# HyperBitGore/deflate.hpp

Measured on AMD Instinct MI355X. Metric: GB/s deflate+inflate on 1 GiB buffer at 1/2/4/8 MI355X; ratio vs reference, higher is better.
Workload: dtype u8; 1 GPU; deflate level 2 + inflate round trip of a per-GPU 1 GiB 'repeat' corpus (SURVEY App. B), device-resident; corpus=repeat, bytes_per_gpu=1073741824, level=2, segment_bytes=32768, parallelism=shard1

## Files before the change

### deflate.hpp_amd/csrc/deflate_kernels.hip

```cpp
#include "dmx_device.h"
#include "dmx_internal.h"
#include "huff_fit.h"

namespace dmx {

constexpr int DF_NT = 1024;
constexpr int DF_CHUNK = 258;
constexpr int df_hash_bits(int seg) {
    return seg >= 32768 ? 12 : 11;
}
constexpr int DF_L3_DEPTH = 16;
constexpr uint32_t DF_L3_LONG = 16;
constexpr uint32_t DF_L3_RP = 512;
constexpr bool df_early(int seg) { return seg >= 32768; }
constexpr uint32_t EM_ALL_LITERALS = 0xFFFFFFFFu;


__device__ __forceinline__ int df_tid() {
    int t = threadIdx.x;
    asm volatile("" : "+v"(t));
    return t;
}

__device__ uint32_t block_excl_scan(uint32_t v, uint32_t* scratch, uint32_t* total) {
// ... 795 lines not shown
                            for (int j = 0; j < 4; j++)
                                x |= __builtin_amdgcn_alignbyte(data32[ip + j + 1], data32[ip + j], sp) ^
                                     __builtin_amdgcn_alignbyte(data32[iq + j + 1], data32[iq + j], sq);
                            pass = x == 0;
                        }
                        const int qb = lane_id() & ~3;
                        uint32_t pm = (uint32_t)(__ballot(pass) >> qb) & 0xFu;
                        while (pm) {
                            const int f = __builtin_ctz(pm);
                            pm &= pm - 1;
                            const uint32_t d1 = (uint32_t)__shfl((int)dk, qb + f, 64);
                            if (len_at(p, d1, ml) >= L) {
                                best = d1;
                                break;
                            }
                        }
                    }
                    if (lead) S.cand[p] = (uint16_t)best;
                }
                tok |= 1u << (p & 31);
                if (lead) S.cand[p + 1] = (uint16_t)L;
                p += L;
            }
            if (tok && lead) atomicOr(&S.tokmap[w], tok);
            if (lead) S.lasttok[t >> 2] = (uint16_t)lastp;
        };
        if (level >= 2 && (uint32_t)t < 4 * nwalk) {
            if constexpr (TERMRUN) {
                if (run_lo != RUN_NONE) parse_walk(std::true_type{});
                else parse_walk(std::false_type{});
            } else
                parse_walk(std::false_type{});
        }
        if constexpr (EARLY) asm volatile("s_waitcnt vmcnt(0)" ::: "memory");
        __syncthreads();
        DMX_PHASE(A.dbg, seg, 3);

        if (level >= 2) {
            const uint32_t sub = t & 3, c = t >> 2;
            const uint32_t hb = D + (c + 1) * CH;
            if ((uint32_t)t < 4 * (nwalk - 1) && hb < nb) {
                const uint32_t s0 = S.lasttok[c], d0 = S.cand[s0], L0 = S.cand[s0 + 1];
                const uint32_t sn = S.lasttok[c + 1];
                if (d0 != 0 && s0 + L0 == hb && L0 < 258 && sn >= hb + 2) {
                    const uint32_t Lx = matchlen4(data32, s0, s0 - d0, min(258u, sn - 1 - s0), sub);
                    const uint32_t e = s0 + Lx;
                    uint32_t q = 0;
                    if (Lx > L0) {
                        uint32_t w = e >> 5;
                        uint32_t m = S.tokmap[w] & (0xFFFFFFFFu >> (31 - (e & 31)));
                        while (!m) m = S.tokmap[--w];
                        q = w * 32 + 31 - (uint32_t)__clz(m);
                    }
                    if (Lx > L0 && sub == 0) {
                        const uint32_t dq = S.cand[q], Lq = q == e ? 0u : S.cand[q + 1];
                        const uint32_t r = q == e ? 0u : q + Lq - e;
                        const uint32_t sync = q == e ? e : q + Lq;
                        uint32_t old = 0;
                        for (uint32_t wi = s0 >> 5; wi <= (sync - 1) >> 5; wi++) {
                            const uint32_t a = max(s0, wi * 32) - wi * 32, z = min(sync, wi * 32 + 32) - wi * 32;
                            const uint32_t rm = (z >= 32 ? 0xFFFFFFFFu : ((1u << z) - 1u)) & (0xFFFFFFFFu << a);
                            old += (uint32_t)__popc(S.tokmap[wi] & rm);
                        }
                        const uint32_t nt = 1 + (r >= 3 ? 1u : r);
                        if (nt < old) {
                            uint32_t nb0 = 0, nb1 = 0;
                            if (r) {
                                atomicOr(&S.tokmap[e >> 5], 1u << (e & 31));
                                if (r == 2) atomicOr(&S.tokmap[(e + 1) >> 5], 1u << ((e + 1) & 31));
                            }
                            S.cand[s0 + 1] = (uint16_t)Lx;
                            if (r >= 3) {
                                S.cand[e] = (uint16_t)dq;
                                S.cand[e + 1] = (uint16_t)r;
                            } else if (r) {
                                S.cand[e] = 0;
                                if (r == 2) S.cand[e + 1] = 0;
                            }
                            for (uint32_t wi = s0 >> 5; wi <= (sync - 1) >> 5; wi++) {
                                const uint32_t a = max(s0, wi * 32) - wi * 32, z = min(sync, wi * 32 + 32) - wi * 32;
                                const uint32_t rm = (z >= 32 ? 0xFFFFFFFFu : ((1u << z) - 1u)) & (0xFFFFFFFFu << a);
                                nb0 = (s0 >> 5) == wi ? 1u << (s0 & 31) : 0u;
                                nb1 = (r && (e >> 5) == wi ? 1u << (e & 31) : 0u) |
                                      (r == 2 && ((e + 1) >> 5) == wi ? 1u << ((e + 1) & 31) : 0u);
                                atomicAnd(&S.tokmap[wi], ~rm | nb0 | nb1);
                            }
                        }
                    }
                }
            }
            __syncthreads();
        }

        bool by_word = false;
        if constexpr (TERMRUN) {
            static_assert(NMAP == DF_NT, "one token-start bitmap word per thread");
            by_word = run_lo != RUN_NONE;
        }
        if (by_word) {
            const uint32_t m = S.tokmap[t];
            const uint4* const c4 = reinterpret_cast<const uint4*>(S.cand + 32 * t);
            uint32_t nz = 0;
#pragma unroll
            for (int k = 0; k < 4; k++) {
                const uint4 v = c4[k];
                const uint32_t x[4] = {v.x, v.y, v.z, v.w};
#pragma unroll
                for (int j = 0; j < 4; j++) {
                    nz |= ((x[j] & 0xFFFFu) ? 1u : 0u) << (8 * k + 2 * j);
                    nz |= ((x[j] >> 16) ? 1u : 0u) << (8 * k + 2 * j + 1);
                }
            }
            const uint32_t mt = m & nz, lt = m & ~nz;
            const uint32_t chain = lt & (lt << 1) & (lt << 2) & (lt << 3);
            uint32_t ws = lt & ~(lt << 1);
#pragma unroll
            for (int i = 0; i < 10; i++) ws |= (ws << 3) & chain;
            const uint32_t val = ((uint32_t)__popc(m) << 16) | ((uint32_t)__popc(mt) + (uint32_t)__popc(ws));
            const uint32_t inc = wave_incl_scan(val);
            uint32_t* const sc = S.scan + DF_NT / 64;
            if ((t & 63) == 63) sc[t >> 6] = inc;
            __syncthreads();
            uint32_t ex = inc - val, tot = 0;
#pragma unroll
            for (int i = 0; i < DF_NT / 64; i++) {
                const uint32_t x = sc[i];
                if (i < (t >> 6)) ex += x;
                tot += x;
            }
            DMX_PHASE(A.dbg, seg, 15);
            if ((tot >> 16) == nb - D) {
                if (t == 0) A.ntok[seg] = EM_ALL_LITERALS;
            } else {
                uint32_t* dst = A.tok + seg * (uint64_t)A.tok_stride + (ex & 0xFFFFu);
                const uint32_t* const sw = reinterpret_cast<const uint32_t*>(&S);
                const uint32_t cbase = (uint32_t)(reinterpret_cast<const uint32_t*>(S.cand) - sw) + 16 * (uint32_t)t;
                const uint32_t dbase = (uint32_t)(data32 - sw) + 8 * (uint32_t)t;
                uint32_t all = mt | ws;
                while (all) {
                    uint32_t b[4], lo[4], hi[4];
                    bool on[4];
#pragma unroll
                    for (int i = 0; i < 4; i++) {
                        on[i] = all != 0;
                        b[i] = on[i] ? (uint32_t)__builtin_ctz(all) : 0u;
                        all &= all - 1;
                        const uint32_t at = (mt >> b[i]) & 1u ? cbase + (b[i] >> 1) : dbase + (b[i] >> 2);
                        lo[i] = sw[at];
                        hi[i] = sw[at + 1];
                    }
#pragma unroll
                    for (int i = 0; i < 4; i++) {
                        if (on[i]) {
                            const bool mat = (mt >> b[i]) & 1u;
                            const uint32_t v = __builtin_amdgcn_alignbyte(hi[i], lo[i], mat ? 2 * (b[i] & 1) : b[i] & 3);
                            const uint32_t x = lt >> b[i], c = 1 + ((x >> 1) & 1u) + ((x >> 1) & (x >> 2) & 1u);
                            *dst++ = mat ? 0x80000000u | (((v >> 16) - 3) << 16) | ((v & 0xFFFFu) - 1)
                                         : (v & (0xFFFFFFu >> (24 - 8 * c))) | (c << 24);
                        }
                    }
                }
                if (t == 0) A.ntok[seg] = tot & 0xFFFFu;
            }
        } else {
            TokRange tr;
            uint32_t tr_total;
            {
                const uint32_t c = t < NMAP ? (uint32_t)__popc(S.tokmap[t]) : 0u;
                uint32_t tot;
                const uint32_t ex = block_excl_scan(c, S.scan, &tot);
                if (t < NMAP) S.mmap[t] = ex;
                __syncthreads();
                tr_total = tot;
                const uint32_t K = (tot + DF_NT - 1) / DF_NT;
                const uint32_t first = min((uint32_t)t * K, tot);
                tr.n = min(first + K, tot) - first;
                uint32_t lo = 0, hi = NMAP;
                while (hi - lo > 1) {
                    const uint32_t mid = (lo + hi) >> 1;
                    if (S.mmap[mid] <= first) lo = mid;
                    else hi = mid;
                }
                tr.w = lo;
                const uint32_t m = S.tokmap[lo];
                uint32_t b = 0, k = tr.n ? first - S.mmap[lo] : 0u;
    #pragma unroll
                for (uint32_t sh = 16; sh >= 1; sh >>= 1) {
                    const uint32_t c = (uint32_t)__popc((m >> b) & ((1u << sh) - 1u));
                    const bool up = k >= c;
                    b += up ? sh : 0u;
                    k -= up ? c : 0u;
                }
                tr.m = m & (0xFFFFFFFFu << b);
            }
            DMX_PHASE(A.dbg, seg, 15);
            const bool all_lit = tr_total == nb - D;
            if (all_lit) {
                if (t == 0) A.ntok[seg] = EM_ALL_LITERALS;
            } else {
                auto walk = [&](auto emit) {
                    uint32_t w = tr.w, m = tr.m, lit = 0, nl = 0;
                    for (uint32_t i = 0; i < tr.n; i++) {
                        const uint32_t p = next_tok(S.tokmap, w, m);
                        const uint32_t d = S.cand[p];
                        if (d) {
                            if (nl) emit(lit | (nl << 24));
                            nl = 0;
                            lit = 0;
                            emit(0x80000000u | ((uint32_t)(S.cand[p + 1] - 3) << 16) | (d - 1));
                        } else {
                            lit |= (uint32_t)data_byte(data32, p) << (8 * nl);
                            if (++nl == 3) {
                                emit(lit | (3u << 24));
                                nl = 0;
                                lit = 0;
                            }
                        }
                    }
                    if (nl) emit(lit | (nl << 24));
                };
                uint32_t nw = 0;
                walk([&](uint32_t) { nw++; });
                uint32_t wtot;
                const uint32_t woff = block_excl_scan(nw, S.scan, &wtot);
                uint32_t* const dst = A.tok + seg * (uint64_t)A.tok_stride + woff;
                uint32_t j = 0;
                walk([&](uint32_t v) { dst[j++] = v; });
                if (t == 0) A.ntok[seg] = wtot;
            }
        }
        DMX_PHASE(A.dbg, seg, 11);
        if constexpr (!EARLY) {
            __syncthreads();
            staged = df_prefetch_next<SEG, BATCH, DICT, PIPE>(A, seg, data32);
        }
        DMX_PHASE(A.dbg, seg, 10);
    }
}

template <int SEG, bool L3, bool BATCH, bool DICT, bool PIPE = false>
__device__ __forceinline__ void deflate_segments(const DeflateArgs& A, DfSmem<SEG>& S) {
    constexpr bool EARLY = DfSmem<SEG>::EARLY;
    uint32_t staged = 0;
    uint32_t iw = 0;
    if constexpr (EARLY) {
        const int t = df_tid();
        if (t < 64) S.buf[t >> 5][SEG / 4 + (t & 31)] = 0;
    }
    uint64_t first = 0;
    if constexpr (PIPE) first = static_cast<const DeflatePipeArgs&>(A).seg_first;
    const auto end = [&]() -> uint64_t {
        if constexpr (PIPE) return static_cast<const DeflatePipeArgs&>(A).seg_end;
        else return df_nseg<BATCH>(A);
    };
    for (uint64_t seg = first + blockIdx.x; seg < end(); seg += gridDim.x) {
        deflate_segment<SEG, L3, BATCH, DICT, PIPE>(A, S, seg, staged, iw);
        if constexpr (EARLY) {
            df_lds_barrier();
            iw = (uint32_t)DfSmem<SEG>::BW - iw;
        } else
            __syncthreads();
    }
}
template <int SEG, bool L3, bool BATCH = false, bool DICT = false>
__global__ __launch_bounds__(DF_NT) void k_deflate_segments(DeflateArgs A) {
    static_assert(!BATCH && !DICT, "a batch runs k_deflate_segments_batch");
    __shared__ DfSmem<SEG> S;
    deflate_segments<SEG, L3, false, false>(A, S);
}
template <bool L3, bool BATCH = false>
__global__ __launch_bounds__(DF_NT) __attribute__((amdgpu_waves_per_eu(8, 8))) void k_deflate_segments16(DeflateArgs A) {
    static_assert(!BATCH, "a batch runs k_deflate_segments16_batch");
    __shared__ DfSmem<16384> S;
    deflate_segments<16384, L3, false, false>(A, S);
}
template <int SEG, bool L3, bool DICT = false>
__global__ __launch_bounds__(DF_NT) void k_deflate_segments_batch(DeflateBatchArgs A) {
    __shared__ DfSmem<SEG> S;
    deflate_segments<SEG, L3, true, DICT>(A, S);
}
template <bool L3>
__global__ __launch_bounds__(DF_NT) __attribute__((amdgpu_waves_per_eu(8, 8))) void k_deflate_segments16_batch(DeflateBatchArgs A) {
    __shared__ DfSmem<16384> S;
    deflate_segments<16384, L3, true, false>(A, S);
}
template <bool L3>
__global__ __launch_bounds__(DF_NT) __attribute__((amdgpu_num_vgpr(52))) void k_deflate_segments_pipe(DeflatePipeArgs A) {
    __shared__ DfSmem<32768> S;
    deflate_segments<32768, L3, false, false, true>(A, S);
}

constexpr int EM_NW = 4;
constexpr int EM_FLUSH = 256;
constexpr int EM_STG = 576;
constexpr int EM_LIT = 288, EM_SYM = 320;

struct EmWave {
    union {
        uint32_t freq[EM_SYM];
        uint32_t stg[EM_STG];
    };
    uint32_t code[EM_SYM];
    uint8_t len[EM_SYM];
    uint16_t rk[EM_SYM];
    uint32_t prefreq[20];
    uint32_t precode[20];
    uint8_t prelen[24];
    uint32_t hcnt[6][20];
    uint32_t lcnt[6][16];
    uint32_t kpre[2][20];
    uint32_t start[2][16];
    uint32_t next[2][16];
};
static_assert(3 * sizeof(EmWave) <= 163840 - 140320, "three emission waves fit beside a front workgroup's LDS");

struct EmCodes {
    uint32_t dyn_tok, fix_tok;
    uint32_t nlit, ndist;
};

__device__ __forceinline__ uint32_t em_slot(int c, int lane) { return c < 5 ? 64 * c + lane : EM_LIT + lane; }
__device__ __forceinline__ bool em_valid(int c, int lane) { return c < 5 ? 64 * c + lane < 286 : lane < 30; }

__device__ EmCodes em_build_codes(EmWave& W) {
    const int lane = lane_id();
    const uint64_t lt = (1ull << lane) - 1ull;
    uint32_t Fl = 0, nzl = 0, hil = 0;
    for (int c = 0; c < 5; c++) {
        const uint32_t f = em_valid(c, lane) ? W.freq[em_slot(c, lane)] : 0u;
        Fl += f;
        const uint64_t b = __ballot(f != 0);
        nzl += (uint32_t)__popcll(b);
        if (b) hil = 64 * c + 64 - (uint32_t)__clzll(b);
    }
    Fl = wave_sum(Fl);
    const uint32_t f5 = lane < 30 ? W.freq[EM_LIT + lane] : 0u;
    const uint32_t Fd = wave_sum(f5);
    const uint64_t bd = __ballot(f5 != 0);
    const uint32_t nzd = (uint32_t)__popcll(bd), hid = bd ? 64 - (uint32_t)__clzll(bd) : 0u;
    for (int c = 0; c < 6; c++) {
        const uint32_t f = em_valid(c, lane) ? W.freq[em_slot(c, lane)] : 0u;
        const uint32_t F = c < 5 ? Fl : Fd;
        const uint32_t L0 = init_len(f, F, c < 5 ? DF_LIT_MAXBITS : DF_DIST_MAXBITS);
        const uint32_t k0 = L0 ? 2 * L0 + init_half(f, F, L0) : 0u;
        uint32_t mine = 0, w0 = 0;
#pragma unroll
        for (int k = 2; k <= 2 * DF_LIT_MAXBITS + 1; k++) {
            const uint64_t b = __ballot(k0 == (uint32_t)k);
            mine = lane == k ? (uint32_t)__popcll(b) : mine;
            w0 = k0 == (uint32_t)k ? (uint32_t)__popcll(b & lt) : w0;
        }
        if (lane < 20) W.hcnt[c][lane] = mine;
        W.rk[64 * c + lane] = (uint16_t)(k0 | (w0 << 5));
    }
    wave_sync();
    {
        const int a = lane >= 32 ? 1 : 0, k = lane & 31;
        uint32_t v = 0;
        if (k < 20) {
            if (a) v = W.hcnt[5][k];
            else v = W.hcnt[0][k] + W.hcnt[1][k] + W.hcnt[2][k] + W.hcnt[3][k] + W.hcnt[4][k];
        }
        uint32_t inc = v;
#pragma unroll
        for (int d = 1; d < 32; d <<= 1) {
            const uint32_t u = __shfl_up(inc, d, 64);
            if (k >= d) inc += u;
        }
        if (k < 20) W.kpre[a][k] = inc - v;
        uint32_t cnt[17];
        cnt[0] = cnt[16] = 0;
        const uint32_t nz = a ? nzd : nzl;
#pragma unroll
        for (int L = 1; L <= 15; L++) {
            const uint32_t x = (2 * L + 1 < 20) ? (uint32_t)__shfl(v, (a << 5) + 2 * L, 64) +
                                                      (uint32_t)__shfl(v, (a << 5) + 2 * L + 1, 64)
                                                : 0u;
            cnt[L] = nz > 1 ? x : (L == 1 ? 2u : 0u);
        }
        if (nz > 1) fit_classes(cnt, a ? DF_DIST_MAXBITS : DF_LIT_MAXBITS);
        if (k == 0) {
            uint32_t st = 0, code = 0;
#pragma unroll
            for (int L = 1; L <= 15; L++) {
                W.start[a][L] = st;
                st += cnt[L];
                code = (code + cnt[L - 1]) << 1;
                W.next[a][L] = code;
            }
        }
    }
    wave_sync();
    for (int c = 0; c < 6; c++) {
        const int a = c == 5 ? 1 : 0;
        const bool sym = em_valid(c, lane);
        const uint32_t nz = a ? nzd : nzl;
        uint32_t L = 0;
        if (sym) {
            const uint32_t s = c < 5 ? 64 * c + lane : (uint32_t)lane;
            if (nz > 1) {
                if (W.freq[em_slot(c, lane)]) {
                    const uint32_t r = W.rk[64 * c + lane], k0 = r & 31;
                    uint32_t q = (r >> 5) + W.kpre[a][k0];
                    for (int c2 = 0; c2 < c && !a; c2++) q += W.hcnt[c2][k0];
#pragma unroll
                    for (int l = 1; l <= 15; l++) L += q >= W.start[a][l] ? 1u : 0u;
                }
            } else {
                const uint32_t u = a ? hid : hil;
                L = (s == (u ? u - 1 : 0u) || s == (u <= 1 ? 1u : 0u)) ? 1u : 0u;
            }
            W.len[em_slot(c, lane)] = (uint8_t)L;
        }
        uint32_t mine = 0, wl = 0;
#pragma unroll
        for (int k = 1; k <= DF_LIT_MAXBITS; k++) {
            const uint64_t b = __ballot(L == (uint32_t)k);
            wl = L == (uint32_t)k ? (uint32_t)__popcll(b & lt) : wl;
            mine = lane == k ? (uint32_t)__popcll(b) : mine;
        }
        if (lane < 16) W.lcnt[c][lane] = mine;
        W.rk[64 * c + lane] = (uint16_t)wl;
    }
    wave_sync();
    uint32_t dyn = 0, fix = 0, hl = 0, hd = 0;
    for (int c = 0; c < 6; c++) {
        const int a = c == 5 ? 1 : 0;
        const bool sym = em_valid(c, lane);
        const uint32_t L = sym ? W.len[em_slot(c, lane)] : 0u;
        if (sym) {
            const uint32_t s = c < 5 ? 64 * c + lane : (uint32_t)lane;
            uint32_t code = 0;
            if (L) {
                uint32_t cc = W.next[a][L] + W.rk[64 * c + lane];
                for (int c2 = 0; c2 < c && !a; c2++) cc += W.lcnt[c2][L];
                code = (L << 16) | bitrev(cc, L);
            }
            W.code[em_slot(c, lane)] = code;
            const uint32_t f = W.freq[em_slot(c, lane)];
            const uint32_t ex = a ? dist_extra(s) : (s > 256 ? len_extra(s) : 0u);
            dyn += f * (L + ex);
            fix += f * ((a ? 5u : fixed_lit_len(s)) + ex);
        }
        const uint64_t used = __ballot(L != 0);
        if (used) {
            const uint32_t h = 64 - (uint32_t)__clzll(used);
            if (a) hd = h;
            else hl = 64 * c + h;
        }
    }
    wave_sync();
    EmCodes r;
    r.dyn_tok = wave_sum(dyn);
    r.fix_tok = wave_sum(fix);
    r.nlit = max(257u, hl);
    r.ndist = max(1u, hd);
    return r;
}

__device__ __forceinline__ void em_put(uint32_t* stg, uint32_t pos, uint64_t pat, uint32_t n) {
    if (!n) return;
    const uint32_t wi = pos >> 5, sh = pos & 31;
    const uint64_t lo = pat << sh;
    atomicOr(&stg[wi], (uint32_t)lo);
    if (sh + n > 32) atomicOr(&stg[wi + 1], (uint32_t)(lo >> 32));
    if (sh + n > 64) atomicOr(&stg[wi + 2], (uint32_t)(pat >> (64 - sh)));
}

__device__ __forceinline__ uint64_t em_pattern(const EmWave& W, uint32_t v, uint32_t cnt, uint32_t& n, bool raw) {
    uint64_t pat = 0;
    n = 0;
    if (!raw && (v >> 31)) {
        const uint32_t L = ((v >> 16) & 0xFFu) + 3, d = (v & 0x7FFFu) + 1;
        const uint32_t ls = len_sym(L), ds = dist_sym(d);
        const uint32_t lc = W.code[ls], dc = W.code[EM_LIT + ds];
        pat = lc & 0xFFFFu;
        n = lc >> 16;
        pat |= (uint64_t)(L - len_base(ls)) << n;
        n += len_extra(ls);
        pat |= (uint64_t)(dc & 0xFFFFu) << n;
        n += dc >> 16;
        pat |= (uint64_t)(d - dist_base(ds)) << n;
        n += dist_extra(ds);
        return pat;
    }
#pragma unroll
    for (uint32_t i = 0; i < 4u; i++) {
        if (i < cnt) {
            const uint32_t c = W.code[(v >> (8 * i)) & 0xFFu];
            pat |= (uint64_t)(c & 0xFFFFu) << n;
            n += c >> 16;
        }
    }
    return pat;
}

__device__ __forceinline__ void em_flush(uint32_t* stg, uint32_t* dst, uint32_t nw) {
    const int lane = lane_id();
#pragma unroll 2
    for (uint32_t i = lane; i < nw; i += 64) dst[i] = stg[i];
    wave_sync();
    const uint32_t part = stg[nw];
    wave_sync();
#pragma unroll 2
    for (uint32_t i = lane; i <= nw + 1; i += 64) stg[i] = i == 0 ? part : 0u;
    wave_sync();
}

#define EM_PHASE(dbg, seg, slot)                                                          \
    do {                                                                                  \
        if ((dbg) && lane_id() == 0) (dbg)[(seg) * kPhaseSlots + (slot)] = __builtin_amdgcn_s_memtime(); \
    } while (0)

struct EmSrc {
    const uint32_t* inw;
    const uint32_t* tok;
    uint64_t in_words_end;
    uint32_t mis;
    uint32_t nb;
    uint32_t ntok;
    bool raw;
    __device__ uint32_t raw_word(uint32_t k) const {
        const uint32_t x = 4 * k + mis;
        const uint32_t a = inw[x >> 2];
        const uint32_t b = (x >> 2) + 1 < in_words_end ? inw[(x >> 2) + 1] : 0u;
        return mis ? __builtin_amdgcn_alignbyte(b, a, x & 3) : a;
    }
    __device__ void load4(uint32_t blk, uint32_t (&v)[4]) const {
        const uint32_t i0 = blk * 256 + 4 * lane_id();
#pragma unroll
        for (int j = 0; j < 4; j++) v[j] = 0;
        if (raw) {
#pragma unroll
            for (int j = 0; j < 4; j++)
                if (i0 + j < ntok) v[j] = raw_word(i0 + j);
        } else if (i0 + 3 < ntok) {
            const uint4 q = *reinterpret_cast<const uint4*>(tok + i0);
            v[0] = q.x, v[1] = q.y, v[2] = q.z, v[3] = q.w;
        } else {
#pragma unroll
            for (int j = 0; j < 4; j++)
                if (i0 + j < ntok) v[j] = tok[i0 + j];
        }
    }
    __device__ uint32_t count_of(uint32_t v, uint32_t idx) const {
        if (raw) return min(4u, nb - 4 * idx);
        return (v >> 31) ? 0u : (v >> 24) & 3u;
    }
};
template <bool RAW>
__device__ EmSrc em_src(const DeflateArgs& A, uint64_t fseg, const uint8_t* inb, uint64_t tail, uint32_t nb) {
    EmSrc s;
    s.mis = (uint32_t)(reinterpret_cast<uintptr_t>(inb) & 3);
    s.inw = reinterpret_cast<const uint32_t*>(inb - s.mis);
    s.in_words_end = (tail + s.mis + 3) / 4;
    s.nb = nb;
    s.raw = RAW || A.ntok[fseg] == EM_ALL_LITERALS;
    s.ntok = s.raw ? (nb + 3) / 4 : A.ntok[fseg];
    s.tok = s.raw ? nullptr : A.tok + fseg * (uint64_t)A.tok_stride;
    return s;
}

__device__ __forceinline__ uint32_t em_stored_hdr(uint32_t q, bool fin, uint32_t len) {
    return q == 0 ? (fin ? 1u : 0u) : q == 1 ? len & 0xFFu : q == 2 ? (len >> 8) & 0xFFu
         : q == 3 ? ~len & 0xFFu : (~len >> 8) & 0xFFu;
}

template <int SEG, bool RAW, bool BATCH>
__device__ void em_segment(const DeflateArgs& A, EmWave& W, uint64_t seg) {
    static_assert(!BATCH || SEG <= 32768, "a batch does not pair front segments into 64 KiB blocks");
    constexpr uint32_t NH = SEG > 32768 ? 2u : 1u;
    constexpr uint32_t HB = (uint32_t)SEG / NH;
    const int lane = lane_id();
    EM_PHASE(A.dbg, seg, 4);
    const DfSegAddr sa = df_seg_addr<SEG, BATCH>(A, seg);
    const uint32_t nb = sa.nb;
    const uint32_t np = (nb + HB - 1) / HB;
    const bool is_final = sa.is_last && A.final_last;
    uint32_t* const slot = reinterpret_cast<uint32_t*>(A.slots + seg * (uint64_t)A.slot_bytes);
    auto part = [&](uint32_t h) {
        return em_src<RAW>(A, seg * NH + h, sa.src + (uint64_t)h * HB, sa.tail - (uint64_t)h * HB, min(HB, nb - h * HB));
    };
    const uint32_t nsto = nb > 65535u ? 2u : 1u;
    const uint32_t n1 = nsto == 2 ? 32768u : nb;
    const uint64_t stored_bytes = 5ull * nsto + nb + (is_final ? 0 : 5);

    if (A.level != 0) {
        for (int i = lane; i < EM_SYM; i += 64) W.freq[i] = 0;
        wave_sync();
        for (uint32_t h = 0; h < np; h++) {
            const EmSrc S = part(h);
            const uint32_t nblk = (S.ntok + 255) / 256;
            for (uint32_t blk = 0; blk < nblk; blk++) {
                uint32_t v[4];
                S.load4(blk, v);
#pragma unroll
                for (int j = 0; j < 4; j++) {
                    const uint32_t idx = blk * 256 + 4 * lane + j;
                    if (idx >= S.ntok) continue;
                    if (!S.raw && (v[j] >> 31)) {
                        atomicAdd(&W.freq[len_sym(((v[j] >> 16) & 0xFFu) + 3)], 1u);
                        atomicAdd(&W.freq[EM_LIT + dist_sym((v[j] & 0x7FFFu) + 1)], 1u);
                    } else {
                        const uint32_t cnt = S.count_of(v[j], idx);
#pragma unroll
                        for (uint32_t i = 0; i < 4u; i++)
                            if (i < cnt) atomicAdd(&W.freq[(v[j] >> (8 * i)) & 0xFFu], 1u);
                    }
                }
            }
        }
        wave_sync();
        if (lane == 0) atomicAdd(&W.freq[256], 1u);
        wave_sync();
        EM_PHASE(A.dbg, seg, 5);
        const EmCodes ec = em_build_codes(W);
        EM_PHASE(A.dbg, seg, 6);
        const uint32_t nlit = ec.nlit, ndist = ec.ndist, nall = nlit + ndist;
        auto seqv = [&](uint32_t i) -> uint32_t { return i < nlit ? W.len[i] : W.len[EM_LIT + i - nlit]; };
        uint64_t rm[5];
        if (lane < 20) W.prefreq[lane] = 0;
#pragma unroll
        for (int c = 0; c < 5; c++) {
            const uint32_t i = 64 * c + lane;
            bool start = false;
            if (i < nall) start = i == 0 || i == nlit || seqv(i - 1) != seqv(i);
            rm[c] = __ballot(start);
        }
        wave_sync();
        for (int c = 0; c < 5; c++) {
            uint32_t rl = 0;
            if ((rm[c] >> lane) & 1) {
                const uint32_t i = 64 * c + lane;
                uint32_t j = nall;
                const uint64_t m = lane < 63 ? rm[c] & (~0ull << (lane + 1)) : 0ull;
                if (m) j = 64 * c + (uint32_t)__builtin_ctzll(m);
                else
                    for (int c2 = 4; c2 > c; c2--)
                        if (rm[c2]) j = 64 * c2 + (uint32_t)__builtin_ctzll(rm[c2]);
                rl = min(j, nall) - i;
                const uint32_t v = seqv(i);
                const RunPlan p = plan_run(v, rl);
                if (p.n18) atomicAdd(&W.prefreq[18], p.n18);
                if (p.n17) atomicAdd(&W.prefreq[17], p.n17);
                if (p.n16) atomicAdd(&W.prefreq[16], p.n16);
                if (p.nlit) atomicAdd(&W.prefreq[v], p.nlit);
            }
            W.rk[64 * c + lane] = (uint16_t)rl;
        }
        wave_sync();
        wave_build_lengths64(W.prefreq, 19, DF_PRE_MAXBITS, W.prelen);
        wave_sync();
        wave_assign_codes(W.prelen, 19, W.precode);
        wave_sync();
        const uint32_t pv = lane < 19 ? W.prelen[kPerm[lane]] : 0u;
        const uint64_t nzp = __ballot(pv != 0u);
        const uint32_t hclen = max(4u, nzp ? 64u - (uint32_t)__clzll(nzp) : 0u);
        uint32_t rtot = 0;
        for (int c = 0; c < 5; c++) {
            const uint32_t rl = W.rk[64 * c + lane];
            uint32_t b = 0;
            if (rl) {
                const uint32_t v = seqv(64 * c + lane);
                const RunPlan p = plan_run(v, rl);
                b = p.n18 * (W.prelen[18] + 7) + p.n17 * (W.prelen[17] + 3) + p.n16 * (W.prelen[16] + 2) +
                    p.nlit * W.prelen[v];
            }
            const uint32_t inc = wave_incl_scan(b);
            W.rk[64 * c + lane] = (uint16_t)(rl ? rtot + inc - b : 0xFFFFu);
            rtot += __shfl(inc, 63, 64);
        }
        wave_sync();
        const uint32_t hdr_bits = 14 + 3 * hclen + rtot;
        EM_PHASE(A.dbg, seg, 7);

        const uint64_t dyn_bits = 3ull + hdr_bits + ec.dyn_tok;
        const uint64_t fix_bits = 3ull + ec.fix_tok;
        const bool use_dyn = dyn_bits <= fix_bits;
        const uint64_t bits = use_dyn ? dyn_bits : fix_bits;
        const uint64_t hbytes = is_final ? (bits + 7) / 8 : (bits + 3 + 7) / 8 + 4;
        if (hbytes < stored_bytes) {
            if (!use_dyn) {
                for (int s = lane; s < EM_SYM; s += 64)
                    W.code[s] = s < EM_LIT ? (s < 286 ? (fixed_lit_len(s) << 16) | fixed_lit_code(s) : 0u)
                                           : (s - EM_LIT < 30 ? (5u << 16) | bitrev(s - EM_LIT, 5) : 0u);
            }
#pragma unroll 3
            for (int i = lane; i < EM_STG; i += 64) W.stg[i] = 0;
            wave_sync();
            if (lane == 0) {
                uint64_t h = (is_final ? 1u : 0u) | ((use_dyn ? 2u : 1u) << 1);
                if (use_dyn) h |= ((uint64_t)(nlit - 257) << 3) | ((uint64_t)(ndist - 1) << 8) | ((uint64_t)(hclen - 4) << 13);
                em_put(W.stg, 0, h, use_dyn ? 17 : 3);
            }
            if (use_dyn) {
                if (lane < (int)hclen) em_put(W.stg, 17 + 3 * lane, pv, 3);
                const uint32_t rb = 17 + 3 * hclen;
                for (int c = 0; c < 5; c++) {
                    const uint32_t ro = W.rk[64 * c + lane];
                    if (ro == 0xFFFFu) continue;
                    const uint32_t i = 64 * c + lane;
                    const uint32_t v = seqv(i);
                    uint32_t j = nall;
                    const uint64_t m = lane < 63 ? rm[c] & (~0ull << (lane + 1)) : 0ull;
                    if (m) j = 64 * c + (uint32_t)__builtin_ctzll(m);
                    else
                        for (int c2 = 4; c2 > c; c2--)
                            if (rm[c2]) j = 64 * c2 + (uint32_t)__builtin_ctzll(rm[c2]);
                    const RunPlan p = plan_run(v, min(j, nall) - i);
                    uint32_t pos = rb + ro;
                    auto put = [&](uint32_t sym, uint32_t extra, uint32_t xb) {
                        const uint32_t pc = W.precode[sym];
                        const uint32_t l = pc >> 16;
                        em_put(W.stg, pos, (uint64_t)(pc & 0xFFFFu) | ((uint64_t)extra << l), l + xb);
                        pos += l + xb;
                    };
                    if (v == 0) {
                        for (uint32_t q = 0; q < p.n18; q++) put(18, (q + 1 == p.n18 ? p.last18 : 138) - 11, 7);
                        if (p.n17) put(17, p.r17 - 3, 3);
                        for (uint32_t q = 0; q < p.nlit; q++) put(0, 0, 0);
                    } else {
                        put(v, 0, 0);
                        for (uint32_t q = 0; q < p.n16; q++) put(16, (q + 1 == p.n16 ? p.last16 : 6) - 3, 2);
                        for (uint32_t q = 1; q < p.nlit; q++) put(v, 0, 0);
                    }
                }
            }
            wave_sync();
            uint32_t cur = 3 + (use_dyn ? hdr_bits : 0u);
            uint32_t* dst = slot;
            for (uint32_t h = 0; h < np; h++) {
                const EmSrc S = part(h);
                const uint32_t nblk = (S.ntok + 255) / 256;
                for (uint32_t blk = 0; blk < nblk; blk++) {
                    uint32_t v[4], nbit[4];
                    uint64_t pat[4];
                    S.load4(blk, v);
                    uint32_t mine = 0;
#pragma unroll
                    for (int j = 0; j < 4; j++) {
                        const uint32_t idx = blk * 256 + 4 * lane + j;
                        nbit[j] = 0;
                        pat[j] = 0;
                        if (idx < S.ntok) pat[j] = em_pattern(W, v[j], S.count_of(v[j], idx), nbit[j], S.raw);
                        mine += nbit[j];
                    }
                    const uint32_t inc = wave_incl_scan(mine);
                    uint32_t pos = cur + inc - mine;
#pragma unroll
                    for (int j = 0; j < 4; j++) {
                        em_put(W.stg, pos, pat[j], nbit[j]);
                        pos += nbit[j];
                    }
                    cur += __shfl(inc, 63, 64);
                    wave_sync();
                    if (cur >= 32u * EM_FLUSH) {
                        const uint32_t nw = cur >> 5;
                        em_flush(W.stg, dst, nw);
                        dst += nw;
                        cur &= 31;
                    }
                }
            }
            EM_PHASE(A.dbg, seg, 8);
            const uint32_t eob = W.code[256];
            if (lane == 0) em_put(W.stg, cur, eob & 0xFFFFu, eob >> 16);
            const uint32_t end_bits = cur + (eob >> 16);
            const uint32_t tail = is_final ? (end_bits + 7) / 8 : (end_bits + 3 + 7) / 8 + 4;
            wave_sync();
            if (lane == 0 && !is_final) {
                atomicOr(&W.stg[(tail - 2) >> 2], 0xFFu << (((tail - 2) & 3) * 8));
                atomicOr(&W.stg[(tail - 1) >> 2], 0xFFu << (((tail - 1) & 3) * 8));
            }
            wave_sync();
            const uint32_t nw = (tail + 3) / 4;
#pragma unroll 2
            for (uint32_t i = lane; i < nw; i += 64) dst[i] = W.stg[i];
            if (lane == 0)
                A.sizes[seg] = (uint32_t)((reinterpret_cast<uint8_t*>(dst) - reinterpret_cast<uint8_t*>(slot)) + tail);
            EM_PHASE(A.dbg, seg, 9);
            return;
        }
    }
    const uint32_t total = (uint32_t)stored_bytes;
    const uint8_t* const inb = sa.src;
    const uint32_t mis = (uint32_t)(reinterpret_cast<uintptr_t>(inb) & 3);
    const uint32_t* const inw = reinterpret_cast<const uint32_t*>(inb - mis);
    const uint64_t in_words_end = (sa.tail + mis + 3) / 4;
    const uint32_t d2 = 10 + n1;
    const uint32_t n16 = (total + 15) / 16;
    uint4* const slot4 = reinterpret_cast<uint4*>(slot);
    auto data_shift = [&](uint32_t a, uint32_t b) -> uint32_t {
        if (a >= 5 && b <= 5 + n1) return 5u;
        if (nsto == 2 && a >= d2 && b <= 10 + nb) return 10u;
        return 0u;
    };
    auto word_at = [&](uint32_t k) -> uint32_t {
        uint32_t w = 0;
        if (const uint32_t sh = data_shift(4 * k, 4 * k + 4)) {
            const uint32_t x = 4 * k - sh + mis;
            const uint32_t a = inw[x >> 2];
            const uint32_t b = (x >> 2) + 1 < in_words_end ? inw[(x >> 2) + 1] : 0u;
            w = __builtin_amdgcn_alignbyte(b, a, x & 3);
        } else {
#pragma unroll
            for (int j = 0; j < 4; j++) {
                const uint32_t pos = 4 * k + j;
                uint32_t byte;
                if (pos < 5) byte = em_stored_hdr(pos, is_final && nsto == 1, n1);
                else if (pos < 5 + n1) byte = inb[pos - 5];
                else if (nsto == 2 && pos < d2) byte = em_stored_hdr(pos - 5 - n1, is_final, nb - n1);
                else if (nsto == 2 && pos < 10 + nb) byte = inb[pos - 10];
                else byte = (!is_final && pos >= 5 * nsto + nb + 3 && pos < total) ? 0xFFu : 0u;
                w |= byte << (8 * j);
            }
        }
        return w;
    };
#pragma unroll 4
    for (uint32_t k4 = lane; k4 < n16; k4 += 64) {
        uint4 o;
        if (const uint32_t sh = data_shift(16 * k4, 16 * k4 + 16)) {
            const uint32_t x = 16 * k4 - sh + mis, i0 = x >> 2, s = x & 3;
            const uint32_t a0 = inw[i0], a1 = inw[i0 + 1], a2 = inw[i0 + 2], a3 = inw[i0 + 3];
            const uint32_t a4 = i0 + 4 < in_words_end ? inw[i0 + 4] : 0u;
            o.x = __builtin_amdgcn_alignbyte(a1, a0, s);
            o.y = __builtin_amdgcn_alignbyte(a2, a1, s);
            o.z = __builtin_amdgcn_alignbyte(a3, a2, s);
            o.w = __builtin_amdgcn_alignbyte(a4, a3, s);
        } else {
            o.x = word_at(4 * k4);
            o.y = word_at(4 * k4 + 1);
            o.z = word_at(4 * k4 + 2);
            o.w = word_at(4 * k4 + 3);
        }
        slot4[k4] = o;
    }
    if (lane == 0) A.sizes[seg] = total;
}

template <int SEG, bool RAW, bool BATCH = false>
__global__ __launch_bounds__(64 * EM_NW) __attribute__((amdgpu_waves_per_eu(6))) void k_deflate_emit(DeflateArgs A) {
    static_assert(!BATCH, "a batch runs k_deflate_emit_batch");
    __shared__ EmWave Ws[EM_NW];
    const uint64_t seg = (uint64_t)blockIdx.x * EM_NW + (threadIdx.x >> 6);
    if (seg >= A.nseg) return;
    em_segment<SEG, RAW, false>(A, Ws[threadIdx.x >> 6], seg);
}
template <int SEG, int NW>
__global__ __launch_bounds__(64 * NW) __attribute__((amdgpu_waves_per_eu(6))) void k_deflate_emit_pipe(DeflatePipeArgs A) {
    __shared__ EmWave Ws[NW];
    const uint64_t seg = A.seg_first + (uint64_t)blockIdx.x * NW + (threadIdx.x >> 6);
    if (seg >= A.seg_end) return;
    em_segment<SEG, false, false>(A, Ws[threadIdx.x >> 6], seg);
}
template <int SEG, bool RAW>
__global__ __launch_bounds__(64 * EM_NW) __attribute__((amdgpu_waves_per_eu(6))) void k_deflate_emit_batch(DeflateBatchArgs A) {
    __shared__ EmWave Ws[EM_NW];
    const uint64_t seg = (uint64_t)blockIdx.x * EM_NW + (threadIdx.x >> 6);
    if (seg >= df_nseg<true>(A)) return;
    em_segment<SEG, RAW, true>(A, Ws[threadIdx.x >> 6], seg);
}

constexpr uint32_t SCAN_NT = 256, SCAN_PER = 32, SCAN_BLK = SCAN_NT * SCAN_PER;
constexpr uint32_t SCAN_ONE = 8;
__device__ __forceinline__ void scan_load32(const uint32_t* v, uint64_t i, uint64_t n, bool vec, uint32_t (&x)[32]) {
    if (vec && i + 32 <= n) {
        const uint4* s4 = reinterpret_cast<const uint4*>(v + i);
#pragma unroll
        for (int k = 0; k < 8; k++) {
            const uint4 q = s4[k];
            x[4 * k] = q.x;
            x[4 * k + 1] = q.y;
            x[4 * k + 2] = q.z;
            x[4 * k + 3] = q.w;
        }
    } else {
#pragma unroll
        for (int k = 0; k < 32; k++) x[k] = i + k < n ? v[i + k] : 0u;
    }
}
__device__ __forceinline__ uint64_t scan_block64(uint64_t s, uint64_t* part, uint64_t* all) {
    const int t = threadIdx.x, lane = t & 63, wave = t >> 6;
    uint64_t inc = s;
#pragma unroll
    for (int d = 1; d < 64; d <<= 1) {
        const uint32_t lo = (uint32_t)__shfl_up((int)(uint32_t)inc, d, 64);
        const uint32_t hi = (uint32_t)__shfl_up((int)(uint32_t)(inc >> 32), d, 64);
        if (lane >= d) inc += ((uint64_t)hi << 32) | lo;
    }
    if (lane == 63) part[wave] = inc;
    __syncthreads();
    uint64_t before = 0, tot = 0;
#pragma unroll
    for (int w = 0; w < (int)(SCAN_NT / 64); w++) {
        const uint64_t v = part[w];
        before += w < wave ? v : 0ull;
        tot += v;
    }
    *all = tot;
    return before + inc;
}
__global__ __launch_bounds__(SCAN_NT) void k_scan_part(const uint32_t* v, uint64_t n, uint64_t* partial) {
    __shared__ uint64_t part[SCAN_NT / 64];
    const uint64_t i = (uint64_t)blockIdx.x * SCAN_BLK + (uint64_t)threadIdx.x * SCAN_PER;
    const bool vec = (reinterpret_cast<uintptr_t>(v) & 15) == 0;
    uint32_t x[32];
    scan_load32(v, i, n, vec, x);
    uint64_t s = 0;
#pragma unroll
    for (int k = 0; k < 32; k++) s += x[k];
    uint64_t all;
    (void)scan_block64(s, part, &all);
    if (threadIdx.x == 0) partial[blockIdx.x] = all;
}
__global__ __launch_bounds__(SCAN_NT) void k_scan_apply(const uint32_t* v, uint64_t n, const uint64_t* partial,
                                                        uint64_t* offs, uint64_t* total, uint64_t* total_host,
                                                        uint64_t* count_dev) {
    __shared__ uint64_t part[SCAN_NT / 64];
    __shared__ uint64_t base_s;
    const int t = threadIdx.x;
    uint64_t pb = 0;
    if (partial) {
        for (uint32_t b = t; b < blockIdx.x; b += SCAN_NT) pb += partial[b];
    } else {
        const bool vecv = (reinterpret_cast<uintptr_t>(v) & 15) == 0;
        for (uint32_t b = 0; b < blockIdx.x; b++) {
            uint32_t y[32];
            scan_load32(v, (uint64_t)b * SCAN_BLK + (uint64_t)t * SCAN_PER, n, vecv, y);
#pragma unroll
            for (int k = 0; k < 32; k++) pb += y[k];
        }
    }
    uint64_t bsum;
    (void)scan_block64(pb, part, &bsum);
    if (t == 0) base_s = bsum;
    __syncthreads();
    const uint64_t base = base_s;
    const uint64_t i = (uint64_t)blockIdx.x * SCAN_BLK + (uint64_t)t * SCAN_PER;
    const bool vec = ((reinterpret_cast<uintptr_t>(v) | reinterpret_cast<uintptr_t>(offs)) & 15) == 0;
    uint32_t x[32];
    scan_load32(v, i, n, vec, x);
    uint64_t s = 0;
#pragma unroll
    for (int k = 0; k < 32; k++) s += x[k];
    uint64_t all;
    uint64_t run = base + scan_block64(s, part, &all) - s;
    uint64_t o[32];
#pragma unroll
    for (int k = 0; k < 32; k++) {
        o[k] = run;
        run += x[k];
    }
    if (vec && i + 32 <= n) {
        ulonglong2* d2 = reinterpret_cast<ulonglong2*>(offs + i);
#pragma unroll
        for (int k = 0; k < 16; k++) d2[k] = make_ulonglong2(o[2 * k], o[2 * k + 1]);
    } else {
#pragma unroll
        for (int k = 0; k < 32; k++)
            if (i + k < n) offs[i + k] = o[k];
    }
    if (blockIdx.x == gridDim.x - 1 && t == 0) {
        *total = base + all;
        if (total_host) *total_host = base + all;
        if (count_dev) *count_dev = base + all + 1;
    }
}

__device__ __forceinline__ void compact_copy(const uint8_t* src, uint8_t* dst, uint32_t sz, uint32_t lane) {
    const uint32_t head = (uint32_t)((4 - ((uintptr_t)dst & 3)) & 3);
    const uint32_t hb = min(head, sz);
    if (lane < hb) dst[lane] = src[lane];
    if (sz <= hb) return;
    const uint32_t rem = sz - hb;
    const uint32_t nw = rem / 4;
    uint32_t* dw = reinterpret_cast<uint32_t*>(dst + hb);
    const uint32_t* sw = reinterpret_cast<const uint32_t*>(src);
    for (uint32_t k = lane; k < nw; k += 64) {
        const uint32_t p = hb + 4 * k;
        dw[k] = __builtin_amdgcn_alignbyte(sw[(p >> 2) + 1], sw[p >> 2], p & 3);
    }
    for (uint32_t i = hb + nw * 4 + lane; i < sz; i += 64) dst[i] = src[i];
}
__global__ __launch_bounds__(256) void k_compact(const uint8_t* slots, uint32_t slot_bytes,
                                                  const uint32_t* sizes, const uint64_t* offs,
                                                  uint64_t nseg, uint8_t* out, uint64_t cap) {
    const uint64_t s = (uint64_t)blockIdx.x * 4 + (threadIdx.x >> 6);
    const uint32_t lane = threadIdx.x & 63;
    if (s >= nseg) return;
    const uint32_t sz = sizes[s];
    const uint64_t o = offs[s];
    const uint8_t* src = slots + s * (uint64_t)slot_bytes;
    if (o + sz > cap) return;
    compact_copy(src, out + o, sz, lane);
}

__global__ __launch_bounds__(256) void k_compact_batch(DeflateBatchArgs A) {
    const uint64_t w = (uint64_t)blockIdx.x * 4 + (threadIdx.x >> 6);
    const uint32_t lane = threadIdx.x & 63;
    if (w < A.nseg) {
        if (w >= df_nseg<true>(A)) return;
        const uint32_t b = A.btab[w].buf & ~DF_BATCH_LAST;
        const uint32_t sz = A.sizes[w];
        const uint64_t rel = A.offsets[w] - A.offsets[A.bfirst[b]];
        if (rel + sz > A.bcap[b]) return;
        compact_copy(A.slots + w * (uint64_t)A.slot_bytes, A.bout[b] + rel, sz, lane);
        return;
    }
    const uint64_t b = (w - A.nseg) * 64 + lane;
    if (b >= A.nbuf) return;
    if (A.bflag && A.bflag[b]) {
        ::dmx_batch_result r;
        r.bytes = 0;
        r.status = DMX_ERR_ARG;
        r.path = 0;
        A.bres[b] = r;
        return;
    }
    const uint64_t s0 = A.bfirst[b], s1 = A.bfirst[b + 1];
    uint64_t bytes;
    if (s0 == s1) {
        bytes = 2;
        if (A.bcap[b] >= 2) {
            A.bout[b][0] = 0x03;
            A.bout[b][1] = 0x00;
        }
    } else {
        bytes = (s1 < A.nseg ? A.offsets[s1] : *A.total) - A.offsets[s0];
    }
    ::dmx_batch_result r;
    r.bytes = bytes;
    r.status = bytes > A.bcap[b] ? DMX_ERR_CAPACITY : DMX_OK;
    r.path = 0;
    A.bres[b] = r;
}

uint64_t deflate_front_fit(uint32_t seg_bytes) {
    int dev = 0, ncu = 0, per = 0;
    (void)hipGetDevice(&dev);
// ... 147 lines not shown
```

Measured before the change: 462.6 GB/s.

## Rebuild emission Huffman code assignment with readlane register counters instead of LDS tables

Rewrites em_build_codes so the per-class histograms, prefix sums, start offsets and next-code values stay in wave registers, read through readlane and ballot loops that visit only the classes present. This removes the hcnt/lcnt/kpre/start/next LDS tables and two wave syncs. It also keeps run-length plans in registers instead of rk, preloads the first token block and reuses it in both passes, clears only the header portion of staging, and makes the segment index scalar. In exchange the code uses more VGPRs and data-dependent loops that may diverge, and the shorter staging clear relies on the header size bound being right.

```diff
diff --git a/deflate.hpp_amd/csrc/deflate_kernels.hip b/deflate.hpp_amd/csrc/deflate_kernels.hip
--- a/deflate.hpp_amd/csrc/deflate_kernels.hip
+++ b/deflate.hpp_amd/csrc/deflate_kernels.hip
@@ -1121,15 +1121,10 @@
     };
     uint32_t code[EM_SYM];
     uint8_t len[EM_SYM];
-    uint16_t rk[EM_SYM];
+    uint16_t rk[6 * 64];
     uint32_t prefreq[20];
     uint32_t precode[20];
     uint8_t prelen[24];
-    uint32_t hcnt[6][20];
-    uint32_t lcnt[6][16];
-    uint32_t kpre[2][20];
-    uint32_t start[2][16];
-    uint32_t next[2][16];
 };
 static_assert(3 * sizeof(EmWave) <= 163840 - 140320, "three emission waves fit beside a front workgroup's LDS");
 
@@ -1141,6 +1136,9 @@
 __device__ __forceinline__ uint32_t em_slot(int c, int lane) { return c < 5 ? 64 * c + lane : EM_LIT + lane; }
 __device__ __forceinline__ bool em_valid(int c, int lane) { return c < 5 ? 64 * c + lane < 286 : lane < 30; }
 
+__device__ __forceinline__ uint32_t em_readlane(uint32_t v, uint32_t l) {
+    return (uint32_t)__builtin_amdgcn_readlane((int)v, (int)l);
+}
 __device__ EmCodes em_build_codes(EmWave& W) {
     const int lane = lane_id();
     const uint64_t lt = (1ull << lane) - 1ull;
@@ -1157,115 +1155,114 @@
     const uint32_t Fd = wave_sum(f5);
     const uint64_t bd = __ballot(f5 != 0);
     const uint32_t nzd = (uint32_t)__popcll(bd), hid = bd ? 64 - (uint32_t)__clzll(bd) : 0u;
+    uint32_t v = 0;
     for (int c = 0; c < 6; c++) {
+        const int a = c == 5 ? 1 : 0;
         const uint32_t f = em_valid(c, lane) ? W.freq[em_slot(c, lane)] : 0u;
-        const uint32_t F = c < 5 ? Fl : Fd;
-        const uint32_t L0 = init_len(f, F, c < 5 ? DF_LIT_MAXBITS : DF_DIST_MAXBITS);
+        uint64_t rem = __ballot(f != 0);
+        if (!rem) continue;
+        const uint32_t F = a ? Fd : Fl;
+        const uint32_t L0 = init_len(f, F, a ? DF_DIST_MAXBITS : DF_LIT_MAXBITS);
         const uint32_t k0 = L0 ? 2 * L0 + init_half(f, F, L0) : 0u;
-        uint32_t mine = 0, w0 = 0;
-#pragma unroll
-        for (int k = 2; k <= 2 * DF_LIT_MAXBITS + 1; k++) {
-            const uint64_t b = __ballot(k0 == (uint32_t)k);
-            mine = lane == k ? (uint32_t)__popcll(b) : mine;
-            w0 = k0 == (uint32_t)k ? (uint32_t)__popcll(b & lt) : w0;
-        }
-        if (lane < 20) W.hcnt[c][lane] = mine;
+        uint32_t w0 = 0;
+        while (rem) {
+            const uint32_t kk = em_readlane(k0, (uint32_t)__builtin_ctzll(rem));
+            const uint64_t b = __ballot(k0 == kk);
+            const uint32_t home = kk + 32 * a;
+            const uint32_t before = em_readlane(v, home);
+            w0 = k0 == kk ? before + (uint32_t)__popcll(b & lt) : w0;
+            v = (uint32_t)lane == home ? before + (uint32_t)__popcll(b) : v;
+            rem &= ~b;
+        }
         W.rk[64 * c + lane] = (uint16_t)(k0 | (w0 << 5));
     }
     wave_sync();
+    uint32_t kp;
+    uint32_t nx = 0;
+    uint32_t stl[DF_LIT_MAXBITS + 1], std_[DF_DIST_MAXBITS + 1];
     {
-        const int a = lane >= 32 ? 1 : 0, k = lane & 31;
-        uint32_t v = 0;
-        if (k < 20) {
-            if (a) v = W.hcnt[5][k];
-            else v = W.hcnt[0][k] + W.hcnt[1][k] + W.hcnt[2][k] + W.hcnt[3][k] + W.hcnt[4][k];
-        }
+        const int k = lane & 31;
         uint32_t inc = v;
 #pragma unroll
         for (int d = 1; d < 32; d <<= 1) {
             const uint32_t u = __shfl_up(inc, d, 64);
             if (k >= d) inc += u;
         }
-        if (k < 20) W.kpre[a][k] = inc - v;
+        kp = inc - v;
+    }
+#pragma unroll
+    for (int a = 0; a < 2; a++) {
+        const int maxbits = a ? DF_DIST_MAXBITS : DF_LIT_MAXBITS;
         uint32_t cnt[17];
         cnt[0] = cnt[16] = 0;
         const uint32_t nz = a ? nzd : nzl;
 #pragma unroll
         for (int L = 1; L <= 15; L++) {
-            const uint32_t x = (2 * L + 1 < 20) ? (uint32_t)__shfl(v, (a << 5) + 2 * L, 64) +
-                                                      (uint32_t)__shfl(v, (a << 5) + 2 * L + 1, 64)
-                                                : 0u;
+            const uint32_t x = L <= maxbits ? em_readlane(v, 32 * a + 2 * L) + em_readlane(v, 32 * a + 2 * L + 1) : 0u;
             cnt[L] = nz > 1 ? x : (L == 1 ? 2u : 0u);
         }
-        if (nz > 1) fit_classes(cnt, a ? DF_DIST_MAXBITS : DF_LIT_MAXBITS);
-        if (k == 0) {
-            uint32_t st = 0, code = 0;
-#pragma unroll
-            for (int L = 1; L <= 15; L++) {
-                W.start[a][L] = st;
-                st += cnt[L];
-                code = (code + cnt[L - 1]) << 1;
-                W.next[a][L] = code;
-            }
-        }
-    }
-    wave_sync();
+        if (nz > 1) fit_classes(cnt, maxbits);
+        uint32_t st = 0, code = 0;
+#pragma unroll
+        for (int L = 1; L <= 15; L++) {
+            if (!a && L <= DF_LIT_MAXBITS) stl[L] = st;
+            if (a && L <= DF_DIST_MAXBITS) std_[L] = st;
+            st += cnt[L];
+            code = (code + cnt[L - 1]) << 1;
+            nx = lane == 32 * a + L ? code : nx;
+        }
+    }
+    uint32_t dyn = 0, fix = 0, hl = 0, hd = 0;
     for (int c = 0; c < 6; c++) {
         const int a = c == 5 ? 1 : 0;
         const bool sym = em_valid(c, lane);
         const uint32_t nz = a ? nzd : nzl;
+        const uint32_t f = sym ? W.freq[em_slot(c, lane)] : 0u;
+        if (nz > 1 && !__ballot(f != 0)) {
+            if (sym) {
+                W.len[em_slot(c, lane)] = 0;
+                W.code[em_slot(c, lane)] = 0;
+            }
+            continue;
+        }
+        const uint32_t s = c < 5 ? 64 * c + lane : (uint32_t)lane;
         uint32_t L = 0;
+        if (nz > 1) {
+            const uint32_t r = W.rk[64 * c + lane];
+            const uint32_t q = (r >> 5) + (uint32_t)__shfl(kp, (int)((r & 31) + 32 * a), 64);
+            uint32_t l = 0;
+#pragma unroll
+            for (int i = 1; i <= DF_LIT_MAXBITS; i++) {
+                const uint32_t st = a ? (i <= DF_DIST_MAXBITS ? std_[i] : 0xFFFFFFFFu) : stl[i];
+                l += q >= st ? 1u : 0u;
+            }
+            L = f ? l : 0u;
+        } else if (sym) {
+            const uint32_t u = a ? hid : hil;
+            L = (s == (u ? u - 1 : 0u) || s == (u <= 1 ? 1u : 0u)) ? 1u : 0u;
+        }
+        if (sym) W.len[em_slot(c, lane)] = (uint8_t)L;
+        uint64_t rem = __ballot(L != 0);
+        if (rem) {
+            const uint32_t h = 64 - (uint32_t)__clzll(rem);
+            if (a) hd = h;
+            else hl = 64 * c + h;
+        }
+        uint32_t cc = 0;
+        while (rem) {
+            const uint32_t kk = em_readlane(L, (uint32_t)__builtin_ctzll(rem));
+            const uint64_t b = __ballot(L == kk);
+            const uint32_t home = kk + 32 * a;
+            const uint32_t first = em_readlane(nx, home);
+            cc = L == kk ? first + (uint32_t)__popcll(b & lt) : cc;
+            nx = (uint32_t)lane == home ? first + (uint32_t)__popcll(b) : nx;
+            rem &= ~b;
+        }
         if (sym) {
-            const uint32_t s = c < 5 ? 64 * c + lane : (uint32_t)lane;
-            if (nz > 1) {
-                if (W.freq[em_slot(c, lane)]) {
-                    const uint32_t r = W.rk[64 * c + lane], k0 = r & 31;
-                    uint32_t q = (r >> 5) + W.kpre[a][k0];
-                    for (int c2 = 0; c2 < c && !a; c2++) q += W.hcnt[c2][k0];
-#pragma unroll
-                    for (int l = 1; l <= 15; l++) L += q >= W.start[a][l] ? 1u : 0u;
-                }
-            } else {
-                const uint32_t u = a ? hid : hil;
-                L = (s == (u ? u - 1 : 0u) || s == (u <= 1 ? 1u : 0u)) ? 1u : 0u;
-            }
-            W.len[em_slot(c, lane)] = (uint8_t)L;
-        }
-        uint32_t mine = 0, wl = 0;
-#pragma unroll
-        for (int k = 1; k <= DF_LIT_MAXBITS; k++) {
-            const uint64_t b = __ballot(L == (uint32_t)k);
-            wl = L == (uint32_t)k ? (uint32_t)__popcll(b & lt) : wl;
-            mine = lane == k ? (uint32_t)__popcll(b) : mine;
-        }
-        if (lane < 16) W.lcnt[c][lane] = mine;
-        W.rk[64 * c + lane] = (uint16_t)wl;
-    }
-    wave_sync();
-    uint32_t dyn = 0, fix = 0, hl = 0, hd = 0;
-    for (int c = 0; c < 6; c++) {
-        const int a = c == 5 ? 1 : 0;
-        const bool sym = em_valid(c, lane);
-        const uint32_t L = sym ? W.len[em_slot(c, lane)] : 0u;
-        if (sym) {
-            const uint32_t s = c < 5 ? 64 * c + lane : (uint32_t)lane;
-            uint32_t code = 0;
-            if (L) {
-                uint32_t cc = W.next[a][L] + W.rk[64 * c + lane];
-                for (int c2 = 0; c2 < c && !a; c2++) cc += W.lcnt[c2][L];
-                code = (L << 16) | bitrev(cc, L);
-            }
-            W.code[em_slot(c, lane)] = code;
-            const uint32_t f = W.freq[em_slot(c, lane)];
+            W.code[em_slot(c, lane)] = L ? (L << 16) | bitrev(cc, L) : 0u;
             const uint32_t ex = a ? dist_extra(s) : (s > 256 ? len_extra(s) : 0u);
             dyn += f * (L + ex);
             fix += f * ((a ? 5u : fixed_lit_len(s)) + ex);
-        }
-        const uint64_t used = __ballot(L != 0);
-        if (used) {
-            const uint32_t h = 64 - (uint32_t)__clzll(used);
-            if (a) hd = h;
-            else hl = 64 * c + h;
         }
     }
     wave_sync();
@@ -1386,8 +1383,10 @@
 }
 
 template <int SEG, bool RAW, bool BATCH>
-__device__ void em_segment(const DeflateArgs& A, EmWave& W, uint64_t seg) {
+__device__ void em_segment(const DeflateArgs& A, EmWave& W, uint64_t seg_of_wave) {
     static_assert(!BATCH || SEG <= 32768, "a batch does not pair front segments into 64 KiB blocks");
+    const uint64_t seg = (uint64_t)(uint32_t)__builtin_amdgcn_readfirstlane((int)(uint32_t)seg_of_wave) |
+                         ((uint64_t)(uint32_t)__builtin_amdgcn_readfirstlane((int)(uint32_t)(seg_of_wave >> 32)) << 32);
     constexpr uint32_t NH = SEG > 32768 ? 2u : 1u;
     constexpr uint32_t HB = (uint32_t)SEG / NH;
     const int lane = lane_id();
@@ -1405,14 +1404,22 @@
     const uint64_t stored_bytes = 5ull * nsto + nb + (is_final ? 0 : 5);
 
     if (A.level != 0) {
+        const EmSrc S0 = part(0);
+        uint32_t v0[4] = {0, 0, 0, 0};
+        if (S0.ntok) S0.load4(0, v0);
         for (int i = lane; i < EM_SYM; i += 64) W.freq[i] = 0;
         wave_sync();
         for (uint32_t h = 0; h < np; h++) {
-            const EmSrc S = part(h);
+            const EmSrc S = h == 0 ? S0 : part(h);
             const uint32_t nblk = (S.ntok + 255) / 256;
             for (uint32_t blk = 0; blk < nblk; blk++) {
                 uint32_t v[4];
-                S.load4(blk, v);
+                if (h == 0 && blk == 0) {
+#pragma unroll
+                    for (int j = 0; j < 4; j++) v[j] = v0[j];
+                } else {
+                    S.load4(blk, v);
+                }
 #pragma unroll
                 for (int j = 0; j < 4; j++) {
                     const uint32_t idx = blk * 256 + 4 * lane + j;
@@ -1447,8 +1454,10 @@
             rm[c] = __ballot(start);
         }
         wave_sync();
+        uint32_t run[5];
+#pragma unroll
         for (int c = 0; c < 5; c++) {
-            uint32_t rl = 0;
+            uint32_t rl = 0, rv = 0;
             if ((rm[c] >> lane) & 1) {
                 const uint32_t i = 64 * c + lane;
                 uint32_t j = nall;
@@ -1459,13 +1468,14 @@
                         if (rm[c2]) j = 64 * c2 + (uint32_t)__builtin_ctzll(rm[c2]);
                 rl = min(j, nall) - i;
                 const uint32_t v = seqv(i);
+                rv = v;
                 const RunPlan p = plan_run(v, rl);
                 if (p.n18) atomicAdd(&W.prefreq[18], p.n18);
                 if (p.n17) atomicAdd(&W.prefreq[17], p.n17);
                 if (p.n16) atomicAdd(&W.prefreq[16], p.n16);
                 if (p.nlit) atomicAdd(&W.prefreq[v], p.nlit);
             }
-            W.rk[64 * c + lane] = (uint16_t)rl;
+            run[c] = rl | (rv << 9);
         }
         wave_sync();
         wave_build_lengths64(W.prefreq, 19, DF_PRE_MAXBITS, W.prelen);
@@ -1476,17 +1486,18 @@
         const uint64_t nzp = __ballot(pv != 0u);
         const uint32_t hclen = max(4u, nzp ? 64u - (uint32_t)__clzll(nzp) : 0u);
         uint32_t rtot = 0;
+        const uint32_t pl16 = W.prelen[16] + 2, pl17 = W.prelen[17] + 3, pl18 = W.prelen[18] + 7;
+#pragma unroll
         for (int c = 0; c < 5; c++) {
-            const uint32_t rl = W.rk[64 * c + lane];
+            const uint32_t rl = run[c] & 511u;
             uint32_t b = 0;
             if (rl) {
-                const uint32_t v = seqv(64 * c + lane);
+                const uint32_t v = run[c] >> 9;
                 const RunPlan p = plan_run(v, rl);
-                b = p.n18 * (W.prelen[18] + 7) + p.n17 * (W.prelen[17] + 3) + p.n16 * (W.prelen[16] + 2) +
-                    p.nlit * W.prelen[v];
+                b = p.n18 * pl18 + p.n17 * pl17 + p.n16 * pl16 + p.nlit * W.prelen[v];
             }
             const uint32_t inc = wave_incl_scan(b);
-            W.rk[64 * c + lane] = (uint16_t)(rl ? rtot + inc - b : 0xFFFFu);
+            if (rl) run[c] |= (rtot + inc - b) << 13;
             rtot += __shfl(inc, 63, 64);
         }
         wave_sync();
@@ -1504,8 +1515,9 @@
                     W.code[s] = s < EM_LIT ? (s < 286 ? (fixed_lit_len(s) << 16) | fixed_lit_code(s) : 0u)
                                            : (s - EM_LIT < 30 ? (5u << 16) | bitrev(s - EM_LIT, 5) : 0u);
             }
+            const uint32_t nclr = min((uint32_t)EM_STG, (uint32_t)((hbytes + 3) / 4) + 1u);
 #pragma unroll 3
-            for (int i = lane; i < EM_STG; i += 64) W.stg[i] = 0;
+            for (uint32_t i = lane; i < nclr; i += 64) W.stg[i] = 0;
             wave_sync();
             if (lane == 0) {
                 uint64_t h = (is_final ? 1u : 0u) | ((use_dyn ? 2u : 1u) << 1);
@@ -1515,19 +1527,13 @@
             if (use_dyn) {
                 if (lane < (int)hclen) em_put(W.stg, 17 + 3 * lane, pv, 3);
                 const uint32_t rb = 17 + 3 * hclen;
+#pragma unroll
                 for (int c = 0; c < 5; c++) {
-                    const uint32_t ro = W.rk[64 * c + lane];
-                    if (ro == 0xFFFFu) continue;
-                    const uint32_t i = 64 * c + lane;
-                    const uint32_t v = seqv(i);
-                    uint32_t j = nall;
-                    const uint64_t m = lane < 63 ? rm[c] & (~0ull << (lane + 1)) : 0ull;
-                    if (m) j = 64 * c + (uint32_t)__builtin_ctzll(m);
-                    else
-                        for (int c2 = 4; c2 > c; c2--)
-                            if (rm[c2]) j = 64 * c2 + (uint32_t)__builtin_ctzll(rm[c2]);
-                    const RunPlan p = plan_run(v, min(j, nall) - i);
-                    uint32_t pos = rb + ro;
+                    const uint32_t rl = run[c] & 511u;
+                    if (!rl) continue;
+                    const uint32_t v = (run[c] >> 9) & 15u;
+                    const RunPlan p = plan_run(v, rl);
+                    uint32_t pos = rb + (run[c] >> 13);
                     auto put = [&](uint32_t sym, uint32_t extra, uint32_t xb) {
                         const uint32_t pc = W.precode[sym];
                         const uint32_t l = pc >> 16;
@@ -1549,12 +1555,17 @@
             uint32_t cur = 3 + (use_dyn ? hdr_bits : 0u);
             uint32_t* dst = slot;
             for (uint32_t h = 0; h < np; h++) {
-                const EmSrc S = part(h);
+                const EmSrc S = h == 0 ? S0 : part(h);
                 const uint32_t nblk = (S.ntok + 255) / 256;
                 for (uint32_t blk = 0; blk < nblk; blk++) {
                     uint32_t v[4], nbit[4];
                     uint64_t pat[4];
-                    S.load4(blk, v);
+                    if (h == 0 && blk == 0) {
+#pragma unroll
+                        for (int j = 0; j < 4; j++) v[j] = v0[j];
+                    } else {
+                        S.load4(blk, v);
+                    }
                     uint32_t mine = 0;
 #pragma unroll
                     for (int j = 0; j < 4; j++) {
```

Result: faster. 475.2 GB/s (median of 6 runs) (+2.7%).
